# thevasudevgupta/gsoc-wav2vec2

Measured on AMD Instinct MI355X. Metric: audio-seconds/s (wav2vec2-base forward, 246000-sample pad), higher is better.
Workload: dtype f32

## Files before the change

gsoc-wav2vec2_amd/csrc/common.h:

```cpp
#pragma once

#include <hip/hip_runtime.h>
#include <stdint.h>
#include <stdio.h>

#include <atomic>

#include <string>

#include "../../include/w2v2.h"

namespace w2v2 {

void set_error(const char* fmt, ...);

#define W2V2_HIP_CHECK(expr)                                                            \
    do {                                                                                \
        hipError_t _e = (expr);                                                         \
        if (_e != hipSuccess) {                                                         \
            ::w2v2::set_error("%s failed: %s (%s:%d)", #expr, hipGetErrorString(_e),    \
                              __FILE__, __LINE__);                                      \
            return W2V2_EHIP;                                                           \
        }                                                                               \
    } while (0)

#define W2V2_REQUIRE(cond, ...)                \
    do {                                       \
        if (!(cond)) {                         \
            ::w2v2::set_error(__VA_ARGS__);    \
            return W2V2_EINVAL;                \
        }                                      \
    } while (0)

#ifdef W2V2_TUNING
int tune_int(const char* name, int dflt);
#else
constexpr int tune_int(const char*, int dflt) { return dflt; }
#endif

__device__ __forceinline__ void grouped_tile(int t, int tiles_m, int tiles_n, int gm, int& tm, int& tn) {
    const int per = gm * tiles_n, grp = t / per, first = grp * gm;
    const int rows = min(gm, tiles_m - first), tl = t - grp * per;
    tn = tl / rows;
    tm = first + (tl - tn * rows);
}
inline int tile_group_rows(int tiles_m, int tiles_n, int64_t a_panel_bytes, int inflight) {
    const int forced = tune_int("W2V2_TILE_GROUP", -1);
    if (forced >= 0) return forced > tiles_m ? tiles_m : forced;
    if (tiles_m < tiles_n || tiles_n < 6) return 0;
    int64_t gm = (int64_t)3407872 / (a_panel_bytes > 0 ? a_panel_bytes : 1);
    const int need = (inflight + tiles_n - 1) / tiles_n;
    if (gm < need) gm = need;
    if (gm < 2) gm = 2;
    const int rows_xcd = (tiles_m + 7) / 8;
    if (gm < rows_xcd) {
        const int ngroups = (int)((rows_xcd + gm - 1) / gm);
        gm = (rows_xcd + ngroups - 1) / ngroups;
    }
    return (int)(gm > tiles_m ? tiles_m : gm);
}

enum Family {
    FAM_CONV0_STATS = 0,
    FAM_CONV0_APPLY,
    FAM_GEMM,
    FAM_GEMM_BF16,
    FAM_GEMM_SPLIT,
    FAM_LAYERNORM,
    FAM_POSCONV,
    FAM_ATTENTION,
    FAM_CTC,
    FAM_MISC,
    FAM_DROPOUT,
    FAM_REDUCE,
    FAM_LN_BWD,
    FAM_OPTIMIZER,
    FAM_COUNT
};
const char* family_name(int f);

enum PlaneFmt { PF_BF16X3 = 0, PF_F16X2 = 1 };
constexpr int plane_count(int fmt) { return fmt == PF_F16X2 ? 2 : 3; }
struct PlaneOut {
    uint16_t* p = nullptr;
    int64_t plane = 0;
    int fmt = PF_BF16X3;
    int* range_flag = nullptr;
};

extern thread_local int tl_launch_family;
void note_kernel_launch();
int64_t kernel_launches(int family);
#define W2V2_LAUNCH(...)                  \
    do {                                  \
        ::w2v2::note_kernel_launch();     \
        hipLaunchKernelGGL(__VA_ARGS__);  \
    } while (0)

struct Profiler;
Profiler* profiler_create();
void profiler_destroy(Profiler*);
void profiler_enable(Profiler*, bool on);
void profiler_set_mask(Profiler*, unsigned family_mask);
void profiler_set_stride(Profiler*, int stride);
int64_t profiler_seen(const Profiler*, int family);
int64_t profiler_kernel_launches(const Profiler*, int family);
bool profiler_enabled(const Profiler*);
void profiler_reset(Profiler*);
int profiler_begin(Profiler*, int family, double flops, double bytes, hipStream_t s);
void profiler_end(Profiler*, int token, hipStream_t s);
int profiler_read(Profiler*, int family, int64_t* launches, double* ms, double* flops, double* bytes);

extern thread_local int tl_prof_depth;
struct ProfScope {
    Profiler* p;
    int tok;
    hipStream_t s;
    int outer_family;
    ProfScope(Profiler* p_, int family, double flops, double bytes, hipStream_t s_)
        : p(p_), tok((p_ && tl_prof_depth == 0) ? profiler_begin(p_, family, flops, bytes, s_) : -1), s(s_), outer_family(tl_launch_family) {
        if (tl_prof_depth++ == 0) tl_launch_family = family;
    }
    ~ProfScope() {
        if (--tl_prof_depth == 0) tl_launch_family = outer_family;
        if (tok >= 0) profiler_end(p, tok, s);
    }
};

extern thread_local Profiler* tl_step_prof;
struct StepProfScope {
    Profiler* outer;
    explicit StepProfScope(Profiler* p) : outer(tl_step_prof) { tl_step_prof = p; }
    ~StepProfScope() { tl_step_prof = outer; }
};

int launch_gemm(Profiler* prof, const float* A, int64_t lda, int64_t strideA, const float* B,
                int64_t ldb, float* C, int64_t ldc, int64_t strideC, const float* bias,
                const float* residual, int M, int N, int K, int nbatch, int act, hipStream_t s);

void gemm_f32_force_ring(int route);
bool gemm_f32_ring_ok(int tile, const float* A, int64_t lda, int64_t strideA, const float* B, int64_t ldb, int64_t strideB,
                      int M, int N, int K);
int launch_gemm_f32_ring(int tile, bool persist, const float* A, int64_t lda, int64_t strideA, const float* B, int64_t ldb,
                         int64_t strideB, float* C, int64_t ldc, int64_t strideC, const float* bias, const float* residual, int M,
                         int N, int K, int nbatch, int act, hipStream_t s);

int launch_gemm_bf16(Profiler* prof, const float* A, int64_t lda, int64_t strideA, const float* B, int64_t ldb,
                     int64_t strideB, float* C, int64_t ldc, int64_t strideC, const float* bias,
                     const float* residual, int M, int N, int K, int nbatch, int act, hipStream_t s);
bool gemm_split_supported(const float* A, int64_t lda, int64_t strideA, int M, int N, int K);
int launch_split_weight(const float* w, uint16_t* planes, int K, int N, hipStream_t s);
int launch_gemm_split(Profiler* prof, const float* A, int64_t lda, int64_t strideA, const uint16_t* planes, float* C, int64_t ldc,
                      int64_t strideC, const float* bias, const float* residual, int M, int N, int K, int nbatch, int act,
                      hipStream_t s);

bool gemm_split_sw_ok(const uint16_t* A16, int64_t planeA, int64_t lda, int64_t strideA, int M, int N, int K);
int launch_split_weight_sw(const float* w, uint16_t* img, int K, int N, int fmt, void* scratch, hipStream_t s);
int launch_split_planes(const float* x, uint16_t* planes, int64_t plane, int64_t n, int fmt, int* range_flag, hipStream_t s);
int launch_gemm_split_sw(Profiler* prof, int fmt, const uint16_t* A16, int64_t planeA, int64_t lda, int64_t strideA, const uint16_t* Bimg,
                         const float* out_scale, float* C, uint16_t* C16, int64_t planeC, int64_t ldc, int64_t strideC, const float* bias,
                         const float* residual, int M, int N, int K, int nbatch, int act, int* range_flag, hipStream_t s);

int launch_check_select_forms(unsigned long long* mismatches_dev , hipStream_t s);

struct GemmShadows {
    const uint16_t* A16 = nullptr;
    const uint16_t* B16 = nullptr;
    uint16_t* C16 = nullptr;
    int64_t ldb16 = 0;
    bool transA = false;
    int zmod = 0;
    int64_t strideB16 = 0, strideC2 = 0, strideBias = 0;
    int64_t strideB2 = 0;
    bool overlapA = false;
    int kseg = 0;
    int64_t segA = 0, segB = 0;
    float* colsum = nullptr;
    int64_t strideCS = 0;
    const uint16_t* B16p = nullptr;
    int64_t validK = 0;
    int kextra = 0;
    bool b_zero_row = false;
    int force_kernel = 0;
};
bool gemm_bf16_sw_ok(int M, int N, int K, int64_t lda, int64_t ldb16, int64_t strideA);
int launch_gemm_bf16_sw(const uint16_t* A16, int64_t lda, int64_t strideA, const uint16_t* B16, int64_t ldb16, float* C, uint16_t* C16,
                        int64_t ldc, int64_t strideC, const float* bias, const float* residual, int M, int N, int K, int nbatch, int act,
                        hipStream_t s);
bool gemm_bf16_swtr_ok(int M, int N, int K, int64_t lda, int64_t ldb, int64_t strideA, int64_t strideB);
int launch_gemm_bf16_swtr(const uint16_t* A16, int64_t lda, int64_t strideA, const uint16_t* B16, int64_t ldb, int64_t strideB, float* C,
                          int64_t ldc, int64_t strideC, int M, int N, int K, int nbatch, hipStream_t s, int kextra = 0, int krag = 0);
bool gemm_bf16_streams_a16(int K, int64_t lda, int64_t strideA);
int launch_gemm_bf16_x(Profiler* prof, const float* A, int64_t lda, int64_t strideA, const float* B, int64_t ldb,
                       int64_t strideB, float* C, int64_t ldc, int64_t strideC, const float* bias,
                       const float* residual, int M, int N, int K, int nbatch, int act, const GemmShadows& x,
                       hipStream_t s);
void gemm_set_precision(int mode);
int gemm_get_precision();
struct PrecisionScope {
    int prev;
    explicit PrecisionScope(int mode) : prev(gemm_get_precision()) { gemm_set_precision(mode); }
    ~PrecisionScope() { gemm_set_precision(prev); }
};
int launch_gemm_ex(Profiler* prof, const float* A, int64_t lda, int64_t strideA, const float* B,
                   int64_t ldb, int64_t strideB, float* C, int64_t ldc, int64_t strideC, const float* bias,
                   const float* residual, int M, int N, int K, int nbatch, int act, hipStream_t s);

int launch_layer_norm(Profiler* prof, const float* x, float* y, const float* gamma,
                      const float* beta, int64_t rows, int C, float eps, int act, hipStream_t s);

int launch_layer_norm_x(Profiler* prof, const float* x, float* y, const float* gamma, const float* beta, int64_t rows,
                        int C, float eps, int act, uint16_t* y16 , hipStream_t s,
                        const PlaneOut* planes = nullptr );

struct PackSeg {
    int64_t s0, len, src0;
    int32_t f0, nf, out0, keep0;
};
struct SegTile {
    int32_t f0, nf, t0, pad;
};
__device__ __forceinline__ int pack_seg_of_sample(const PackSeg* segs, int n, int64_t pos) {
    int lo = 0, hi = n - 1;
    while (lo < hi) {
        const int mid = (lo + hi + 1) >> 1;
        if (segs[mid].s0 <= pos) lo = mid; else hi = mid - 1;
    }
    return lo;
}

int64_t conv0_ws_floats(int B, int64_t L, int K, int stride, int C);
int conv0_chunk_frames();
int launch_conv0_packed(Profiler* prof, const float* wave, const float* kernel, const float* bias, const float* gamma,
                        const float* beta, float* out, float* ws, float* scale_shift, int64_t L, int K, int stride, int C,
                        float eps, int act, const PackSeg* segs, int nseg, hipStream_t s,
                        const PlaneOut* planes = nullptr ,
                        double* gram_ws = nullptr ,
                        int max_seg_frames = 0 );
int64_t conv0_gram_ws_doubles(int64_t L, int stride, int nseg);
int launch_conv0(Profiler* prof, const float* wave, const float* kernel, const float* bias,
                 const float* gamma, const float* beta, float* out, float* ws, int B, int64_t L,
                 int K, int stride, int C, float eps, int norm_mode, int act, hipStream_t s);

int launch_conv0_x(Profiler* prof, const float* wave, const float* kernel, const float* bias,
                   const float* gamma, const float* beta, float* out, uint16_t* out16 , float* ws,
                   int B, int64_t L, int K, int stride, int C, float eps, int norm_mode, int act, hipStream_t s,
                   const PlaneOut* planes = nullptr );
int launch_to_bf16(const float* x, uint16_t* y, int64_t n, hipStream_t s);
struct ShadowJob {
    const float* w;
    uint16_t* wt;
    uint16_t* plain;
    int K, N, k0, n0;
};
int launch_weight_shadows_multi(const ShadowJob* jobs_dev, int njobs, hipStream_t s);
int launch_transpose_to_bf16(const float* w, uint16_t* wt, int K, int N, hipStream_t s);
int launch_transpose_to_bf16_batched(const float* w, uint16_t* wt, int K, int N, int nbatch, hipStream_t s);

int launch_weight_norm_regroup(Profiler* prof, const float* wv, const float* wg, float* out, int K,
                               int cg, int H, int groups, hipStream_t s);
int launch_pos_conv(Profiler* prof, const float* x, const float* wg, const float* bias,
                    const int32_t* frame_len, float* y, int B, int T, int H, int K, int groups,
                    int act, hipStream_t s);

int64_t pos_conv_bf16_pack_elems(int B, int T, int H, int K);
int launch_pos_conv_weight_shadow(const float* wg, uint16_t* w16, int K, int cg, int groups, hipStream_t s);
int launch_pos_conv_bf16(Profiler* prof, const float* x, const uint16_t* w16, const float* bias, const int32_t* frame_len,
                         float* y, float* pre_act, uint16_t* pack16, float* xz_ws, int B, int T, int H, int K, int groups,
                         int act, int pad_left, int add_residual, hipStream_t s);

int launch_pos_conv_dw_bf16(Profiler* prof, const float* xz, const float* dc, float* dwg, float* pack32, float* slabs, float* red_ws,
                            int B, int T, int H, int K, int groups, hipStream_t s, float* dc_pad = nullptr );

int launch_attention(Profiler* prof, const float* qkv, const int32_t* frame_len, float* ctx, int B,
                     int T, int H, int heads, hipStream_t s);

int pos_conv_packed_rows();
int launch_pos_conv_packed(Profiler* prof, const float* x, const float* wg, const float* bias, float* y, const SegTile* tiles,
                           int ntiles, int64_t frames, int H, int K, int groups, int act, hipStream_t s);
int attention_packed_rows(int head_size);
int launch_attention_packed(Profiler* prof, const float* qkv, float* ctx, const SegTile* tiles, int ntiles, int64_t frames,
                            double sum_nf2, int H, int heads, hipStream_t s);
int launch_pack_scatter(const float* src, float* stream, int64_t L, const PackSeg* segs, int nseg, hipStream_t s,
                        const double* stats = nullptr);
int launch_pack_stats(const float* src, const PackSeg* segs, int nseg, double eps, double* stats, hipStream_t s);
int launch_pack_gather(const float* stream_rows, float* out, int64_t out_rows, int width, const PackSeg* segs, int nseg,
                       hipStream_t s);
int launch_pack_zero_gaps(float* x, const PlaneOut* pl, int64_t frames, int width, const PackSeg* segs, int nseg, hipStream_t s);

enum ScratchSlot { SCRATCH_SPLITK = 0, SCRATCH_CTC = 1, SCRATCH_QKV16 = 2, SCRATCH_DCTX16 = 3, SCRATCH_ALIGN = 4, SCRATCH_BEAM = 5, SCRATCH_WINDOWS = 6,
                   SCRATCH_CUTS = 7 };
int stream_scratch(int slot, hipStream_t s, size_t bytes, void** out);
int stream_scratch_release();
struct PinnedStage {
    void* p = nullptr;
    size_t bytes = 0;
    hipEvent_t copied = nullptr;
};
// ... 206 lines not shown
```

gsoc-wav2vec2_amd/csrc/gemm_f32.hip:

```cpp
#include <stdlib.h>


#include "common.h"
#include "gemm_epilogue.h"

namespace w2v2 {

using f32x16 = __attribute__((ext_vector_type(16))) float;
using f32x4 = __attribute__((ext_vector_type(4))) float;

namespace {

constexpr int BK = 32;
constexpr int LDA_S = BK + 4;

struct GemmArgs {
    const float* A;
    const float* B;
    float* C;
    const float* bias;
    const float* residual;
    int64_t lda, ldb, ldc, strideA, strideB, strideC;
    int M, N, K, act;
    int tiles_m, tiles_n;
// ... 258 lines not shown
    __syncthreads();
    for (int kt = 0; kt + 1 < nk; ++kt) {
        const int cur = kt & 1;
        issue_tile(kt + 1, cur ^ 1);
        __builtin_amdgcn_sched_barrier(0);
        compute(cur);
        __builtin_amdgcn_sched_barrier(0);
        __syncthreads();
    }
    compute((nk - 1) & 1);

    {
        const int64_t tile_off = (int64_t)z * g.strideC + (int64_t)(m0 + wm * WTM) * g.ldc + (n0 + wn * WTN);
        gemm_epilogue<MT, NTL, false>(acc, g.C + tile_off, nullptr, g.residual ? g.residual + tile_off : nullptr,
                                     g.bias ? g.bias + (n0 + wn * WTN) : nullptr, (int)g.ldc, g.M - (m0 + wm * WTM),
                                     g.N - (n0 + wn * WTN), g.act, li, lh);
    }
}

template <int WM, int WN, int MINW, int BKT = 32, int BM = 128, int BN = 128>
int launch_dma(GemmArgs& g, int nbatch, hipStream_t s) {
    g.tiles_m = (g.M + BM - 1) / BM;
    g.tiles_n = (g.N + BN - 1) / BN;
    dim3 grid(g.tiles_m * g.tiles_n, 1, nbatch), block(WM * WN * 64);
    const size_t lds = 2 * (BM * BKT + BKT * BN) * sizeof(float);
    const int per_cu = (int)(160 * 1024 / lds) < 1 ? 1 : (int)(160 * 1024 / lds) > 4 ? 4 : (int)(160 * 1024 / lds);
    g.gm = nbatch == 1 ? tile_group_rows(g.tiles_m, g.tiles_n, (int64_t)BM * g.K * 4, 32 * per_cu) : 0;
    static std::atomic<bool> attr_set{false};
    if (!attr_set && lds > 64 * 1024) {
        W2V2_HIP_CHECK(hipFuncSetAttribute(reinterpret_cast<const void*>(gemm_f32_dma_kernel<WM, WN, MINW, BKT, BM, BN>),
                                           hipFuncAttributeMaxDynamicSharedMemorySize, (int)lds));
        attr_set = true;
    }
    W2V2_LAUNCH((gemm_f32_dma_kernel<WM, WN, MINW, BKT, BM, BN>), grid, block, lds, s, g);
    W2V2_HIP_CHECK(hipGetLastError());
    return W2V2_OK;
}

template <int BM, int BN, int WM, int WN, int MINW>
int launch_cfg(GemmArgs& g, bool fast, int nbatch, hipStream_t s) {
    using C_ = Cfg<BM, BN, WM, WN>;
    g.tiles_m = (g.M + BM - 1) / BM;
    g.tiles_n = (g.N + BN - 1) / BN;
    static std::atomic<bool> attr_set{false};
    if (!attr_set) {
        W2V2_HIP_CHECK(hipFuncSetAttribute(reinterpret_cast<const void*>(gemm_f32_kernel<true, BM, BN, WM, WN, MINW>),
                                           hipFuncAttributeMaxDynamicSharedMemorySize, (int)C_::LDS));
        W2V2_HIP_CHECK(hipFuncSetAttribute(reinterpret_cast<const void*>(gemm_f32_kernel<false, BM, BN, WM, WN, MINW>),
                                           hipFuncAttributeMaxDynamicSharedMemorySize, (int)C_::LDS));
        attr_set = true;
    }
    dim3 grid(g.tiles_m * g.tiles_n, 1, nbatch), block(C_::NT);
    if (fast)
        W2V2_LAUNCH((gemm_f32_kernel<true, BM, BN, WM, WN, MINW>), grid, block, C_::LDS, s, g);
    else
        W2V2_LAUNCH((gemm_f32_kernel<false, BM, BN, WM, WN, MINW>), grid, block, C_::LDS, s, g);
    W2V2_HIP_CHECK(hipGetLastError());
    return W2V2_OK;
}

int forced_cfg() {
    return tune_int("W2V2_GEMM_CFG", -1);
}

__global__ __launch_bounds__(256) void splitk_reduce_kernel(const float* __restrict__ slabs, float* __restrict__ C, const float* __restrict__ bias,
                                                            const float* __restrict__ residual, int M, int N, int64_t ldc, int S, int act) {
    const int64_t n4 = (int64_t)M * N / 4;
    for (int64_t i = (int64_t)blockIdx.x * 256 + threadIdx.x; i < n4; i += (int64_t)gridDim.x * 256) {
        const int64_t e = i * 4, row = e / N;
        const int col = (int)(e % N);
        float4 acc = reinterpret_cast<const float4*>(slabs)[i];
        for (int z = 1; z < S; ++z) {
            const float4 v = reinterpret_cast<const float4*>(slabs + (int64_t)z * M * N)[i];
            acc.x += v.x; acc.y += v.y; acc.z += v.z; acc.w += v.w;
        }
        if (bias) { acc.x += bias[col]; acc.y += bias[col + 1]; acc.z += bias[col + 2]; acc.w += bias[col + 3]; }
        acc.x = apply_act(acc.x, act); acc.y = apply_act(acc.y, act); acc.z = apply_act(acc.z, act); acc.w = apply_act(acc.w, act);
        if (residual) {
            const float4 r = *reinterpret_cast<const float4*>(residual + row * ldc + col);
            acc.x += r.x; acc.y += r.y; acc.z += r.z; acc.w += r.w;
        }
        *reinterpret_cast<float4*>(C + row * ldc + col) = acc;
    }
}

thread_local int tl_precision = 0;
thread_local int tl_ring = -1;

constexpr int RING_DEFAULT = 2;
int ring_route() { return tl_ring >= 0 ? tl_ring : tune_int("W2V2_GEMM_RING", RING_DEFAULT); }

}

void gemm_set_precision(int mode) { tl_precision = mode; }
void gemm_f32_force_ring(int route) { tl_ring = route; }
int gemm_get_precision() { return tl_precision; }

int launch_gemm(Profiler* prof, const float* A, int64_t lda, int64_t strideA, const float* B,
                int64_t ldb, float* C, int64_t ldc, int64_t strideC, const float* bias,
                const float* residual, int M, int N, int K, int nbatch, int act, hipStream_t s) {
    return launch_gemm_ex(prof, A, lda, strideA, B, ldb, 0, C, ldc, strideC, bias, residual, M, N, K, nbatch, act, s);
}

int launch_gemm_ex(Profiler* prof, const float* A, int64_t lda, int64_t strideA, const float* B,
                   int64_t ldb, int64_t strideB, float* C, int64_t ldc, int64_t strideC, const float* bias,
                   const float* residual, int M, int N, int K, int nbatch, int act, hipStream_t s) {
    if (tl_precision == 1)
        return launch_gemm_bf16(prof, A, lda, strideA, B, ldb, strideB, C, ldc, strideC, bias, residual, M, N, K, nbatch, act, s);
    W2V2_REQUIRE(A && B && C, "gemm: null operand");
    W2V2_REQUIRE(M > 0 && N > 0 && K > 0 && nbatch > 0, "gemm: bad sizes M=%d N=%d K=%d batch=%d", M, N, K, nbatch);
    W2V2_REQUIRE(lda >= 1 && ldb >= N && ldc >= N && ldc < (1 << 23), "gemm: bad leading dimensions");
    W2V2_REQUIRE(act >= 0 && act <= 2, "gemm: bad activation %d", act);
    GemmArgs g;
    g.A = A; g.B = B; g.C = C; g.bias = bias; g.residual = residual;
    g.lda = lda; g.ldb = ldb; g.ldc = ldc; g.strideA = strideA; g.strideB = strideB; g.strideC = strideC;
    g.M = M; g.N = N; g.K = K; g.act = act;
    const bool fast = (K % BK == 0) && (N % 4 == 0) && (lda % 4 == 0) && (ldb % 4 == 0) &&
                      (strideA % 4 == 0) && (strideB % 4 == 0) && ((reinterpret_cast<uintptr_t>(A) & 15) == 0) &&
                      ((reinterpret_cast<uintptr_t>(B) & 15) == 0);
    ProfScope ps(prof, FAM_GEMM, 2.0 * M * (double)N * K * nbatch,
                 4.0 * nbatch * ((double)M * K + (double)M * N) + 4.0 * (double)K * N, s);
    int cfg = forced_cfg();
    const bool by_shape = cfg < 0;
    if (cfg < 0 && fast && nbatch == 1 && strideB == 0 && K >= 1024 && (ldc % 4) == 0 &&
        ((reinterpret_cast<uintptr_t>(C) | reinterpret_cast<uintptr_t>(residual) | reinterpret_cast<uintptr_t>(bias)) & 15) == 0) {
        const int64_t tiles64 = (int64_t)((M + 63) / 64) * ((N + 63) / 64);
        int S = 1;
        for (int cand = 8; cand >= 2; cand >>= 1)
            if (K % (cand * BK) == 0 && K / cand >= 256 && tiles64 * cand <= 512) { S = cand; break; }
        if (S > 1 && tiles64 <= 256) {
            const size_t need = (size_t)S * M * N;
            float* ws = nullptr;
            void* raw = nullptr;
            if (int e = stream_scratch(SCRATCH_SPLITK, s, need * sizeof(float), &raw)) return e;
            ws = reinterpret_cast<float*>(raw);
            GemmArgs h = g;
            h.C = ws; h.bias = nullptr; h.residual = nullptr; h.act = 0;
            h.K = K / S; h.strideA = K / S; h.strideB = (int64_t)(K / S) * ldb; h.ldc = N; h.strideC = (int64_t)M * N;
            if (int e = launch_dma<2, 2, 2, 32, 64, 64>(h, S, s)) return e;
            const int64_t n4 = (int64_t)M * N / 4;
            int64_t blocks = (n4 + 255) / 256;
            blocks = blocks > 2048 ? 2048 : blocks;
            W2V2_LAUNCH(splitk_reduce_kernel, dim3((unsigned)blocks), dim3(256), 0, s, ws, C, bias, residual, M, N, ldc, S, act);
            W2V2_HIP_CHECK(hipGetLastError());
            return W2V2_OK;
        }
    }
    if (cfg < 0) {
        cfg = 7;
        const int64_t tiles128 = (int64_t)((M + 127) / 128) * ((N + 127) / 128) * nbatch;
        if (fast && tiles128 < 384) cfg = 16;
        const int tail_knob = tune_int("W2V2_GEMM_TAIL", 1);
        const int64_t tn = (N + 127) / 128, S = 512, r = tiles128 % S;
        if (tail_knob && fast && cfg == 7 && nbatch == 1 && tiles128 > S && r != 0 && 4 * r <= S) {
            const int64_t main_rows = ((tiles128 - r) / tn) * 128;
            if (main_rows > 0 && main_rows < M) {
                GemmArgs h = g;
                h.M = (int)main_rows;
                const int ring = by_shape ? ring_route() : 0;
                if (ring && strideB == 0 && gemm_f32_ring_ok(1, A, lda, strideA, B, ldb, strideB, h.M, N, K)) {
                    if (int e = launch_gemm_f32_ring(1, ring == 2, A, lda, strideA, B, ldb, strideB, C, ldc, strideC, bias, residual,
                                                     h.M, N, K, 1, act, s))
                        return e;
                } else if (int e = launch_dma<2, 4, 2>(h, 1, s)) {
                    return e;
                }
                GemmArgs t = g;
                t.A = g.A + main_rows * lda;
                t.C = g.C + main_rows * ldc;
                t.residual = g.residual ? g.residual + main_rows * ldc : nullptr;
                t.M = M - (int)main_rows;
                return launch_dma<2, 2, 2, 32, 64, 64>(t, 1, s);
            }
        }
    }
    const int wide_min = tune_int("W2V2_GEMM_WIDE", 1536);
    if (cfg == 7 && fast && wide_min > 0 && N % 128 == 0) {
        const int64_t tm256 = (M + 255) / 256, tiles256 = tm256 * (N / 128) * nbatch;
        if (tiles256 >= wide_min && (tm256 * 256 - M) * 40 <= M) {
            const int ring = by_shape ? ring_route() : 0;
            if (ring && strideB == 0 && gemm_f32_ring_ok(0, A, lda, strideA, B, ldb, strideB, M, N, K))
                return launch_gemm_f32_ring(0, ring == 2, A, lda, strideA, B, ldb, strideB, C, ldc, strideC, bias, residual, M, N, K,
                                            nbatch, act, s);
            return launch_dma<4, 2, 2, 16, 256, 128>(g, nbatch, s);
        }
    }
    if (cfg == 7 && fast) {
        const int ring = by_shape ? ring_route() : 0;
        if (ring && strideB == 0 && gemm_f32_ring_ok(1, A, lda, strideA, B, ldb, strideB, M, N, K))
            return launch_gemm_f32_ring(1, ring == 2, A, lda, strideA, B, ldb, strideB, C, ldc, strideC, bias, residual, M, N, K,
                                        nbatch, act, s);
    }
    switch (cfg) {
        case 16: if (fast) return launch_dma<2, 2, 2, 32, 64, 64>(g, nbatch, s); return launch_cfg<128, 128, 2, 2, 2>(g, fast, nbatch, s);
        case 14: if (fast) return launch_dma<2, 3, 2, 32, 128, 96>(g, nbatch, s); return launch_cfg<128, 128, 2, 2, 2>(g, fast, nbatch, s);
        case 1: return launch_cfg<128, 256, 2, 2, 1>(g, fast, nbatch, s);
        case 2: return launch_cfg<256, 128, 2, 2, 1>(g, fast, nbatch, s);
        case 3: return launch_cfg<256, 256, 4, 2, 2>(g, fast, nbatch, s);
        case 4: if (fast) return launch_dma<2, 2, 2>(g, nbatch, s); return launch_cfg<128, 128, 2, 2, 2>(g, fast, nbatch, s);
        case 6: if (fast) return launch_dma<4, 2, 2>(g, nbatch, s); return launch_cfg<128, 128, 2, 2, 2>(g, fast, nbatch, s);
        case 7: if (fast) return launch_dma<2, 4, 2>(g, nbatch, s); return launch_cfg<128, 128, 2, 2, 2>(g, fast, nbatch, s);
        case 9: if (fast) return launch_dma<2, 4, 3, 16>(g, nbatch, s); return launch_cfg<128, 128, 2, 2, 2>(g, fast, nbatch, s);
        case 10: if (fast) return launch_dma<2, 4, 4, 16>(g, nbatch, s); return launch_cfg<128, 128, 2, 2, 2>(g, fast, nbatch, s);
        case 11: if (fast) return launch_dma<2, 2, 4, 16>(g, nbatch, s); return launch_cfg<128, 128, 2, 2, 2>(g, fast, nbatch, s);
        case 12: if (fast && g.N >= 256) return launch_dma<4, 4, 1, 32, 256, 256>(g, nbatch, s); return launch_cfg<128, 128, 2, 2, 2>(g, fast, nbatch, s);
        case 13: if (fast && g.N >= 128) return launch_dma<4, 2, 1, 32, 256, 128>(g, nbatch, s); return launch_cfg<128, 128, 2, 2, 2>(g, fast, nbatch, s);
        case 8: if (fast) return launch_dma<4, 4, 1>(g, nbatch, s); return launch_cfg<128, 128, 2, 2, 2>(g, fast, nbatch, s);
#ifdef W2V2_TUNING
        case 17: if (fast && g.N >= 256) return launch_dma<2, 4, 2, 16, 128, 256>(g, nbatch, s); return launch_dma<2, 4, 2>(g, nbatch, s);
        case 18: if (fast && g.N >= 128) return launch_dma<4, 2, 2, 16, 256, 128>(g, nbatch, s); return launch_dma<2, 4, 2>(g, nbatch, s);
        case 19: if (fast && g.N >= 256) return launch_dma<2, 4, 2, 32, 128, 256>(g, nbatch, s); return launch_dma<2, 4, 2>(g, nbatch, s);
#endif
        default: return launch_cfg<128, 128, 2, 2, 2>(g, fast, nbatch, s);
    }
}

}
```

gsoc-wav2vec2_amd/csrc/gemm_f32_sw.hip:

```cpp
#include "common.h"
#include "gemm_epilogue.h"
#include "gemm_sw_common.h"

namespace w2v2 {

namespace {

struct GemmRingArgs {
    const float* A;
    const float* B;
    float* C;
    const float* bias;
    const float* residual;
    int64_t lda, ldb, ldc, strideA, strideB, strideC;
    int M, N, K, act;
    int tiles_m, tiles_n, nbatch;
    int gm;
};

template <int WM, int WN, int BKT, int BM, int BN, int NS>
struct RingCfg {
    static constexpr int STAGE = (BM * BKT + BKT * BN) * 4;
    static constexpr int LDS = NS * STAGE;
    static constexpr int NW = WM * WN;
    static constexpr int NPA = BM * BKT / 256, NPB = BKT * BN / 256;
    static constexpr int PPA = NPA / NW, PPB = NPB / NW;
    static constexpr int P = PPA + PPB;
    static_assert(NPA % NW == 0 && NPB % NW == 0, "every wave issues the same number of pieces (counted waits)");
    static_assert((NS - 2) * P <= 63, "vmcnt field");
};

template <int WM, int WN, int BKT, int BM, int BN, int NS>
__global__ __launch_bounds__(WM* WN * 64) __attribute__((amdgpu_waves_per_eu(4))) void gemm_f32_ring_kernel(GemmRingArgs g) {
    using R_ = RingCfg<WM, WN, BKT, BM, BN, NS>;
    constexpr int NW = R_::NW, PPA = R_::PPA, PPB = R_::PPB, P = R_::P, STAGE = R_::STAGE;
    constexpr int RPP = 256 / BKT;
    constexpr int SPR = BKT / 4;
    constexpr int SW = BKT == 32 ? 1 : 2;
    constexpr int WTM = BM / WM, WTN = BN / WN, MT = WTM / 32, NTL = WTN / 32;
    extern __shared__ __attribute__((aligned(16))) float smem[];
    const int tid = threadIdx.x, lane = tid & 63, wave = __builtin_amdgcn_readfirstlane(tid >> 6);
    const int wm = wave / WN, wn = wave % WN, li = lane & 31, lh = lane >> 5;
    const unsigned lds0 = (unsigned)(uintptr_t)(__attribute__((address_space(3))) float*)smem;

    const int nwg = g.tiles_m * g.tiles_n, total = nwg * g.nbatch, G = gridDim.x;
    const int ntl = (total - (int)blockIdx.x + G - 1) / G;
    const int nk = g.K / BKT, nsteps = ntl * nk;
    auto tile_of = [&](int i, int& z, int& m0, int& n0) {
        const int v = (int)blockIdx.x + i * G;
        const int q = total >> 3, r = total & 7, xcd = v & 7, idx = v >> 3;
        int t = (xcd < r ? xcd * (q + 1) : r * (q + 1) + (xcd - r) * q) + idx;
        z = t / nwg;
        t -= z * nwg;
        int tm = t / g.tiles_n, tn = t % g.tiles_n;
        if (g.gm > 0) grouped_tile(t, g.tiles_m, g.tiles_n, g.gm, tm, tn);
        m0 = tm * BM;
        n0 = tn * BN;
    };

    int ii = 0, ikt = 0, ist = 0;
    const unsigned char* baseA = nullptr;
    const unsigned char* baseB = nullptr;
    uint32_t offA[PPA], offB[PPB];
    auto uniform_ptr = [](const void* p) {
        const uint64_t v = reinterpret_cast<uint64_t>(p);
        const uint32_t lo = __builtin_amdgcn_readfirstlane((uint32_t)v), hi = __builtin_amdgcn_readfirstlane((uint32_t)(v >> 32));
        return reinterpret_cast<const unsigned char*>(((uint64_t)hi << 32) | lo);
    };
    auto set_issue_tile = [&](int i) {
        int z, m0, n0;
        tile_of(i, z, m0, n0);
        baseA = uniform_ptr(g.A + (int64_t)z * g.strideA + (int64_t)m0 * g.lda);
        baseB = uniform_ptr(g.B + (int64_t)z * g.strideB + n0);
#pragma unroll
        for (int p = 0; p < PPA; ++p) {
            const int r = (wave + p * NW) * RPP + lane / SPR;
            const int rr = m0 + r < g.M ? r : g.M - 1 - m0;
            const int slot = (lane % SPR) ^ ((r >> SW) & (SPR - 1));
            offA[p] = (uint32_t)((int64_t)rr * g.lda * 4) + (uint32_t)slot * 16u;
        }
#pragma unroll
        for (int p = 0; p < PPB; ++p) {
            const int flat = (wave + p * NW) * 256 + lane * 4;
            const int br = flat / BN, c = flat % BN;
            const int cc = n0 + c < g.N ? c : g.N - 4 - n0;
            offB[p] = (uint32_t)((int64_t)br * g.ldb * 4) + (uint32_t)cc * 4u;
        }
    };
    auto issue_step = [&]() {
        const unsigned dst = lds0 + (unsigned)ist * STAGE;
        const unsigned char* a = baseA + (int64_t)ikt * BKT * 4;
        const unsigned char* b = baseB + (int64_t)ikt * BKT * g.ldb * 4;
#pragma unroll
        for (int p = 0; p < PPA; ++p) sw_dma(dst + (unsigned)(wave + p * NW) * 1024u, offA[p], a);
#pragma unroll
        for (int p = 0; p < PPB; ++p) sw_dma(dst + (unsigned)(BM * BKT * 4) + (unsigned)(wave + p * NW) * 1024u, offB[p], b);
        ist = ist + 1 == NS ? 0 : ist + 1;
        if (++ikt == nk) {
            ikt = 0;
            if (++ii < ntl) set_issue_tile(ii);
        }
    };

    f32x16 acc[MT][NTL];
    auto zero = [&]() {
#pragma unroll
        for (int i = 0; i < MT; ++i)
#pragma unroll
            for (int j = 0; j < NTL; ++j)
#pragma unroll
                for (int r = 0; r < 16; ++r) acc[i][j][r] = 0.0f;
    };
    int a_row[MT], a_swz[MT];
#pragma unroll
    for (int mt = 0; mt < MT; ++mt) {
        const int i = wm * WTM + mt * 32 + li;
        a_row[mt] = i * BKT;
        a_swz[mt] = (i >> SW) & (SPR - 1);
    }
    auto compute = [&](int stage) {
        const float* As = smem + stage * (STAGE / 4);
        const float* Bs = As + BM * BKT + (4 * lh) * BN + wn * WTN + li;
#pragma unroll
        for (int kb = 0; kb < BKT / 8; ++kb) {
            f32x4 a[MT];
            float b[NTL][4];
#pragma unroll
            for (int mt = 0; mt < MT; ++mt)
                a[mt] = *reinterpret_cast<const f32x4*>(As + a_row[mt] + (((2 * kb + lh) ^ a_swz[mt]) << 2));
#pragma unroll
            for (int nt = 0; nt < NTL; ++nt)
#pragma unroll
                for (int e = 0; e < 4; ++e) b[nt][e] = Bs[(kb * 8 + e) * BN + nt * 32];
#pragma unroll
            for (int e = 0; e < 4; ++e)
#pragma unroll
                for (int mt = 0; mt < MT; ++mt)
#pragma unroll
                    for (int nt = 0; nt < NTL; ++nt)
                        acc[mt][nt] = __builtin_amdgcn_mfma_f32_32x32x2f32(a[mt][e], b[nt][e], acc[mt][nt], 0, 0, 0);
        }
    };
    auto ring_barrier = [&](bool counted) {
        if (counted) sw_wait_vm<(NS - 2) * P>();
        else sw_wait_vm<0>();
        __builtin_amdgcn_s_barrier();
        asm volatile("" ::: "memory");
        __builtin_amdgcn_sched_barrier(0);
    };

    set_issue_tile(0);
    for (int p = 0; p < NS - 1 && p < nsteps; ++p) issue_step();
    ring_barrier(nsteps >= NS - 1);
    __builtin_amdgcn_s_setprio(1);

    int s = 0, cst = 0;
    for (int ci = 0; ci < ntl; ++ci) {
        zero();
        for (int kt = 0; kt < nk; ++kt, ++s) {
            const bool more = s + NS - 1 < nsteps;
            if (more) issue_step();
            __builtin_amdgcn_sched_barrier(0);
            compute(cst);
            __builtin_amdgcn_sched_barrier(0);
            ring_barrier(more);
            cst = cst + 1 == NS ? 0 : cst + 1;
        }
        int z, m0, n0;
        tile_of(ci, z, m0, n0);
        const int64_t tile_off = (int64_t)z * g.strideC + (int64_t)(m0 + wm * WTM) * g.ldc + (n0 + wn * WTN);
        int act = g.act, ldc = (int)g.ldc, eli = li, elh = lh;
        const float* res = g.residual;
        const float* bias = g.bias;
        asm volatile("" : "+s"(act), "+s"(res), "+s"(bias), "+s"(ldc), "+v"(eli), "+v"(elh));
        __builtin_amdgcn_s_setprio(0);
        gemm_epilogue<MT, NTL, false>(acc, g.C + tile_off, nullptr, res ? res + tile_off : nullptr, bias ? bias + (n0 + wn * WTN) : nullptr,
                                     ldc, g.M - (m0 + wm * WTM), g.N - (n0 + wn * WTN), act, eli, elh);
        __builtin_amdgcn_s_setprio(1);
    }
    __builtin_amdgcn_s_setprio(0);
}

template <int WM, int WN, int BKT, int BM, int BN, int NS>
int launch_ring(GemmRingArgs& g, bool persist, hipStream_t s) {
    using R_ = RingCfg<WM, WN, BKT, BM, BN, NS>;
    static_assert(2 * R_::LDS <= 160 * 1024, "two blocks per CU");
    g.tiles_m = (g.M + BM - 1) / BM;
    g.tiles_n = (g.N + BN - 1) / BN;
    const int64_t total = (int64_t)g.tiles_m * g.tiles_n * g.nbatch;
    W2V2_REQUIRE(total < (1ll << 31), "gemm ring: %lld tiles", (long long)total);
    int grid = (int)total;
    if (persist) {
        int dev = 0, cus = 0;
        W2V2_HIP_CHECK(hipGetDevice(&dev));
        W2V2_HIP_CHECK(hipDeviceGetAttribute(&cus, hipDeviceAttributeMultiprocessorCount, dev));
        const int resident = (2 * cus) & ~7;
        if (resident >= 8 && total > resident) grid = resident;
    }
    g.gm = g.nbatch == 1 ? tile_group_rows(g.tiles_m, g.tiles_n, (int64_t)BM * g.K * 4, BM == 256 ? 96 : 64) : 0;
    static std::atomic<bool> attr_set{false};
    if (!attr_set) {
        W2V2_HIP_CHECK(hipFuncSetAttribute(reinterpret_cast<const void*>(gemm_f32_ring_kernel<WM, WN, BKT, BM, BN, NS>),
                                           hipFuncAttributeMaxDynamicSharedMemorySize, R_::LDS));
        attr_set = true;
    }
    W2V2_LAUNCH((gemm_f32_ring_kernel<WM, WN, BKT, BM, BN, NS>), dim3(grid), dim3(WM * WN * 64), R_::LDS, s, g);
    W2V2_HIP_CHECK(hipGetLastError());
    return W2V2_OK;
}

}

bool gemm_f32_ring_ok(int tile, const float* A, int64_t lda, int64_t strideA, const float* B, int64_t ldb, int64_t strideB,
                      int M, int N, int K) {
    const int BM = tile == 0 ? 256 : 128, BKT = 16;
    const bool align = ((reinterpret_cast<uintptr_t>(A) | reinterpret_cast<uintptr_t>(B)) & 15) == 0 && lda % 4 == 0 &&
                       ldb % 4 == 0 && strideA % 4 == 0 && strideB % 4 == 0;
    return align && K % BKT == 0 && N % 4 == 0 && N >= 4 && (int64_t)BM * lda * 4 < (1ll << 31) &&
           (int64_t)BKT * ldb * 4 < (1ll << 31) && M > 0;
}

int launch_gemm_f32_ring(int tile, bool persist, const float* A, int64_t lda, int64_t strideA, const float* B, int64_t ldb,
                         int64_t strideB, float* C, int64_t ldc, int64_t strideC, const float* bias, const float* residual, int M,
                         int N, int K, int nbatch, int act, hipStream_t s) {
    W2V2_REQUIRE(tile == 0 || tile == 1, "gemm ring: tile %d", tile);
    W2V2_REQUIRE(gemm_f32_ring_ok(tile, A, lda, strideA, B, ldb, strideB, M, N, K), "gemm ring: unsupported shape M=%d N=%d K=%d", M, N, K);
    GemmRingArgs g;
    g.A = A; g.B = B; g.C = C; g.bias = bias; g.residual = residual;
    g.lda = lda; g.ldb = ldb; g.ldc = ldc; g.strideA = strideA; g.strideB = strideB; g.strideC = strideC;
    g.M = M; g.N = N; g.K = K; g.act = act; g.nbatch = nbatch;
    if (tile == 0) return launch_ring<4, 2, 16, 256, 128, 3>(g, persist, s);
    return launch_ring<2, 4, 16, 128, 128, 4>(g, persist, s);
}

}
```

Baseline: 8155.

## Add 64x64 ring GEMM tile and split wave-tail tiles into quarter tiles

Adds a smaller 64x64, BK=32 ring-GEMM configuration and uses it for small GEMMs (cfg 16) and for the row tail of the tail-split path. It also adds a flat split launch. The first 128x128 tiles in grouped order run as a normal ring kernel, and the leftover wave-tail tiles are each split into four 64x64 quarter tiles in a second launch. The goal is to cut the partial last wave and improve CU balance. In exchange it adds an extra launch and smaller tiles with less reuse, and changes persistent residency and grouping heuristics.

Result: faster. 8304, median of 6 (+1.8%).

```diff
diff --git a/gsoc-wav2vec2_amd/csrc/common.h b/gsoc-wav2vec2_amd/csrc/common.h
--- a/gsoc-wav2vec2_amd/csrc/common.h
+++ b/gsoc-wav2vec2_amd/csrc/common.h
@@ -144,6 +144,8 @@
 int launch_gemm_f32_ring(int tile, bool persist, const float* A, int64_t lda, int64_t strideA, const float* B, int64_t ldb,
                          int64_t strideB, float* C, int64_t ldc, int64_t strideC, const float* bias, const float* residual, int M,
                          int N, int K, int nbatch, int act, hipStream_t s);
+int launch_gemm_f32_ring_split(bool persist, int64_t main_tiles, const float* A, int64_t lda, const float* B, int64_t ldb, float* C,
+                               int64_t ldc, const float* bias, const float* residual, int M, int N, int K, int act, hipStream_t s);
 
 int launch_gemm_bf16(Profiler* prof, const float* A, int64_t lda, int64_t strideA, const float* B, int64_t ldb,
                      int64_t strideB, float* C, int64_t ldc, int64_t strideC, const float* bias,
diff --git a/gsoc-wav2vec2_amd/csrc/gemm_f32.hip b/gsoc-wav2vec2_amd/csrc/gemm_f32.hip
--- a/gsoc-wav2vec2_amd/csrc/gemm_f32.hip
+++ b/gsoc-wav2vec2_amd/csrc/gemm_f32.hip
@@ -434,8 +434,12 @@
         if (fast && tiles128 < 384) cfg = 16;
         const int tail_knob = tune_int("W2V2_GEMM_TAIL", 1);
         const int64_t tn = (N + 127) / 128, S = 512, r = tiles128 % S;
-        if (tail_knob && fast && cfg == 7 && nbatch == 1 && tiles128 > S && r != 0 && 4 * r <= S) {
+        if (tail_knob && fast && cfg == 7 && nbatch == 1 && tiles128 > S && r != 0 && tune_int("W2V2_GEMM_TAIL_DIV", 4) * r <= S) {
             const int64_t main_rows = ((tiles128 - r) / tn) * 128;
+            const int ring_flat = by_shape && tune_int("W2V2_GEMM_TAIL_FLAT", 1) ? ring_route() : 0;
+            if (ring_flat && strideB == 0 && M % 128 == 0 && N % 128 == 0 && gemm_f32_ring_ok(1, A, lda, 0, B, ldb, 0, M, N, K) &&
+                gemm_f32_ring_ok(2, A, lda, 0, B, ldb, 0, M, N, K))
+                return launch_gemm_f32_ring_split(ring_flat == 2, tiles128 - r, A, lda, B, ldb, C, ldc, bias, residual, M, N, K, act, s);
             if (main_rows > 0 && main_rows < M) {
                 GemmArgs h = g;
                 h.M = (int)main_rows;
@@ -452,9 +456,18 @@
                 t.C = g.C + main_rows * ldc;
                 t.residual = g.residual ? g.residual + main_rows * ldc : nullptr;
                 t.M = M - (int)main_rows;
+                if (ring && strideB == 0 && gemm_f32_ring_ok(2, t.A, lda, strideA, B, ldb, strideB, t.M, N, K))
+                    return launch_gemm_f32_ring(2, ring == 2, t.A, lda, strideA, B, ldb, strideB, t.C, ldc, strideC, bias,
+                                                t.residual, t.M, N, K, 1, act, s);
                 return launch_dma<2, 2, 2, 32, 64, 64>(t, 1, s);
             }
         }
+    }
+    if (cfg == 16 && fast && by_shape) {
+        const int ring = ring_route();
+        if (ring && strideB == 0 && gemm_f32_ring_ok(2, A, lda, strideA, B, ldb, strideB, M, N, K))
+            return launch_gemm_f32_ring(2, ring == 2, A, lda, strideA, B, ldb, strideB, C, ldc, strideC, bias, residual, M, N, K,
+                                        nbatch, act, s);
     }
     const int wide_min = tune_int("W2V2_GEMM_WIDE", 1536);
     if (cfg == 7 && fast && wide_min > 0 && N % 128 == 0) {
diff --git a/gsoc-wav2vec2_amd/csrc/gemm_f32_sw.hip b/gsoc-wav2vec2_amd/csrc/gemm_f32_sw.hip
--- a/gsoc-wav2vec2_amd/csrc/gemm_f32_sw.hip
+++ b/gsoc-wav2vec2_amd/csrc/gemm_f32_sw.hip
@@ -16,6 +16,8 @@
     int M, N, K, act;
     int tiles_m, tiles_n, nbatch;
     int gm;
+    int total;
+    int first;
 };
 
 template <int WM, int WN, int BKT, int BM, int BN, int NS>
@@ -30,7 +32,7 @@
     static_assert((NS - 2) * P <= 63, "vmcnt field");
 };
 
-template <int WM, int WN, int BKT, int BM, int BN, int NS>
+template <int WM, int WN, int BKT, int BM, int BN, int NS, bool QUAD = false>
 __global__ __launch_bounds__(WM* WN * 64) __attribute__((amdgpu_waves_per_eu(4))) void gemm_f32_ring_kernel(GemmRingArgs g) {
     using R_ = RingCfg<WM, WN, BKT, BM, BN, NS>;
     constexpr int NW = R_::NW, PPA = R_::PPA, PPB = R_::PPB, P = R_::P, STAGE = R_::STAGE;
@@ -43,19 +45,28 @@
     const int wm = wave / WN, wn = wave % WN, li = lane & 31, lh = lane >> 5;
     const unsigned lds0 = (unsigned)(uintptr_t)(__attribute__((address_space(3))) float*)smem;
 
-    const int nwg = g.tiles_m * g.tiles_n, total = nwg * g.nbatch, G = gridDim.x;
+    const int nwg = g.tiles_m * g.tiles_n, total = g.total, G = gridDim.x;
     const int ntl = (total - (int)blockIdx.x + G - 1) / G;
     const int nk = g.K / BKT, nsteps = ntl * nk;
     auto tile_of = [&](int i, int& z, int& m0, int& n0) {
         const int v = (int)blockIdx.x + i * G;
         const int q = total >> 3, r = total & 7, xcd = v & 7, idx = v >> 3;
         int t = (xcd < r ? xcd * (q + 1) : r * (q + 1) + (xcd - r) * q) + idx;
+        int sub = 0;
+        if constexpr (QUAD) {
+            sub = t & 3;
+            t = g.first + (t >> 2);
+        }
         z = t / nwg;
         t -= z * nwg;
         int tm = t / g.tiles_n, tn = t % g.tiles_n;
         if (g.gm > 0) grouped_tile(t, g.tiles_m, g.tiles_n, g.gm, tm, tn);
         m0 = tm * BM;
         n0 = tn * BN;
+        if constexpr (QUAD) {
+            m0 = 2 * m0 + (sub >> 1) * BM;
+            n0 = 2 * n0 + (sub & 1) * BN;
+        }
     };
 
     int ii = 0, ikt = 0, ist = 0;
@@ -181,30 +192,37 @@
     __builtin_amdgcn_s_setprio(0);
 }
 
-template <int WM, int WN, int BKT, int BM, int BN, int NS>
-int launch_ring(GemmRingArgs& g, bool persist, hipStream_t s) {
+template <int WM, int WN, int BKT, int BM, int BN, int NS, bool QUAD = false>
+int launch_ring(GemmRingArgs& g, bool persist, hipStream_t s, int64_t first = -1, int gm = 0) {
     using R_ = RingCfg<WM, WN, BKT, BM, BN, NS>;
     static_assert(2 * R_::LDS <= 160 * 1024, "two blocks per CU");
-    g.tiles_m = (g.M + BM - 1) / BM;
-    g.tiles_n = (g.N + BN - 1) / BN;
-    const int64_t total = (int64_t)g.tiles_m * g.tiles_n * g.nbatch;
+    constexpr int TM = QUAD ? 2 * BM : BM, TN = QUAD ? 2 * BN : BN;
+    g.tiles_m = (g.M + TM - 1) / TM;
+    g.tiles_n = (g.N + TN - 1) / TN;
+    int64_t total = (int64_t)g.tiles_m * g.tiles_n * g.nbatch;
+    W2V2_REQUIRE(first < 0 || (first > 0 && first < total && g.nbatch == 1 && g.M % TM == 0 && g.N % TN == 0), "gemm ring: bad split");
+    W2V2_REQUIRE(!QUAD || first > 0, "gemm ring: quarter tiles need a split");
+    g.first = QUAD ? (int)first : 0;
+    if (first > 0) total = QUAD ? 4 * (total - first) : first;
     W2V2_REQUIRE(total < (1ll << 31), "gemm ring: %lld tiles", (long long)total);
+    g.total = (int)total;
+    constexpr int PER_CU = WM * WN == 8 ? 2 : 160 * 1024 / R_::LDS > 4 ? 4 : 160 * 1024 / R_::LDS;
     int grid = (int)total;
     if (persist) {
         int dev = 0, cus = 0;
         W2V2_HIP_CHECK(hipGetDevice(&dev));
         W2V2_HIP_CHECK(hipDeviceGetAttribute(&cus, hipDeviceAttributeMultiprocessorCount, dev));
-        const int resident = (2 * cus) & ~7;
+        const int resident = (PER_CU * cus) & ~7;
         if (resident >= 8 && total > resident) grid = resident;
     }
-    g.gm = g.nbatch == 1 ? tile_group_rows(g.tiles_m, g.tiles_n, (int64_t)BM * g.K * 4, BM == 256 ? 96 : 64) : 0;
+    g.gm = first > 0 ? gm : g.nbatch == 1 ? tile_group_rows(g.tiles_m, g.tiles_n, (int64_t)BM * g.K * 4, BM == 256 ? 96 : 32 * PER_CU) : 0;
     static std::atomic<bool> attr_set{false};
     if (!attr_set) {
-        W2V2_HIP_CHECK(hipFuncSetAttribute(reinterpret_cast<const void*>(gemm_f32_ring_kernel<WM, WN, BKT, BM, BN, NS>),
+        W2V2_HIP_CHECK(hipFuncSetAttribute(reinterpret_cast<const void*>(gemm_f32_ring_kernel<WM, WN, BKT, BM, BN, NS, QUAD>),
                                            hipFuncAttributeMaxDynamicSharedMemorySize, R_::LDS));
         attr_set = true;
     }
-    W2V2_LAUNCH((gemm_f32_ring_kernel<WM, WN, BKT, BM, BN, NS>), dim3(grid), dim3(WM * WN * 64), R_::LDS, s, g);
+    W2V2_LAUNCH((gemm_f32_ring_kernel<WM, WN, BKT, BM, BN, NS, QUAD>), dim3(grid), dim3(WM * WN * 64), R_::LDS, s, g);
     W2V2_HIP_CHECK(hipGetLastError());
     return W2V2_OK;
 }
@@ -213,7 +231,7 @@
 
 bool gemm_f32_ring_ok(int tile, const float* A, int64_t lda, int64_t strideA, const float* B, int64_t ldb, int64_t strideB,
                       int M, int N, int K) {
-    const int BM = tile == 0 ? 256 : 128, BKT = 16;
+    const int BM = tile == 0 ? 256 : tile == 1 ? 128 : 64, BKT = tile == 2 ? 32 : 16;
     const bool align = ((reinterpret_cast<uintptr_t>(A) | reinterpret_cast<uintptr_t>(B)) & 15) == 0 && lda % 4 == 0 &&
                        ldb % 4 == 0 && strideA % 4 == 0 && strideB % 4 == 0;
     return align && K % BKT == 0 && N % 4 == 0 && N >= 4 && (int64_t)BM * lda * 4 < (1ll << 31) &&
@@ -223,14 +241,28 @@
 int launch_gemm_f32_ring(int tile, bool persist, const float* A, int64_t lda, int64_t strideA, const float* B, int64_t ldb,
                          int64_t strideB, float* C, int64_t ldc, int64_t strideC, const float* bias, const float* residual, int M,
                          int N, int K, int nbatch, int act, hipStream_t s) {
-    W2V2_REQUIRE(tile == 0 || tile == 1, "gemm ring: tile %d", tile);
+    W2V2_REQUIRE(tile >= 0 && tile <= 2, "gemm ring: tile %d", tile);
     W2V2_REQUIRE(gemm_f32_ring_ok(tile, A, lda, strideA, B, ldb, strideB, M, N, K), "gemm ring: unsupported shape M=%d N=%d K=%d", M, N, K);
     GemmRingArgs g;
     g.A = A; g.B = B; g.C = C; g.bias = bias; g.residual = residual;
     g.lda = lda; g.ldb = ldb; g.ldc = ldc; g.strideA = strideA; g.strideB = strideB; g.strideC = strideC;
     g.M = M; g.N = N; g.K = K; g.act = act; g.nbatch = nbatch;
     if (tile == 0) return launch_ring<4, 2, 16, 256, 128, 3>(g, persist, s);
-    return launch_ring<2, 4, 16, 128, 128, 4>(g, persist, s);
-}
-
-}
+    if (tile == 1) return launch_ring<2, 4, 16, 128, 128, 4>(g, persist, s);
+    return launch_ring<2, 2, 32, 64, 64, 3>(g, persist, s);
+}
+
+int launch_gemm_f32_ring_split(bool persist, int64_t main_tiles, const float* A, int64_t lda, const float* B, int64_t ldb, float* C,
+                               int64_t ldc, const float* bias, const float* residual, int M, int N, int K, int act, hipStream_t s) {
+    W2V2_REQUIRE(M % 128 == 0 && N % 128 == 0 && gemm_f32_ring_ok(1, A, lda, 0, B, ldb, 0, M, N, K) && gemm_f32_ring_ok(2, A, lda, 0, B, ldb, 0, M, N, K),
+                 "gemm ring split: unsupported shape M=%d N=%d K=%d", M, N, K);
+    GemmRingArgs g;
+    g.A = A; g.B = B; g.C = C; g.bias = bias; g.residual = residual;
+    g.lda = lda; g.ldb = ldb; g.ldc = ldc; g.strideA = 0; g.strideB = 0; g.strideC = 0;
+    g.M = M; g.N = N; g.K = K; g.act = act; g.nbatch = 1;
+    const int gm = tile_group_rows(M / 128, N / 128, (int64_t)128 * K * 4, 64);
+    if (int e = launch_ring<2, 4, 16, 128, 128, 4>(g, persist, s, main_tiles, gm)) return e;
+    return launch_ring<2, 2, 32, 64, 64, 3, true>(g, false, s, main_tiles, gm);
+}
+
+}
```
